# zerchen/AlignSDF

Measured on AMD Instinct MI355X. Metric: meshes_per_sec_hand_plus_obj_N256, higher is better.
Workload: dtype f32-class: 2 x f16 planes per operand (22 bit), 3 f16 MFMAs per product sum, f32 accumulate, every voxel <= 1e-5

## Files before the change

### alignsdf_amd/csrc/decoder.hip

```cpp
#include <hip/hip_runtime.h>

#include <cstdlib>
#include <cstring>
#include <new>
#include <vector>

#include "../../include/alignsdf_hip.h"
#include "common.h"
#include "pack.h"
#include "k1_launch.h"
#include "fold_kernels.h"
#include "sweep_kernels.h"

namespace asdf {
thread_local int g_last_hip_error = 0;
}

using namespace asdf;

struct asdf_decoder {
  asdf_decoder_spec_t spec;
  int device;
  int num_cus;
  float* stream;
  float* wlat;
  float* wpt;
  float* bias02;
  float* cst;
  int kp;
  float* embed;
  float* latent_stage;
  float* cls;
  int num_class;
  float* stream16;
  float* stream16_hi;
  float* cst16;
  float* a16;
  float* cst16p1;
  float* cst16p1_host;
  uint16_t* hi_host;
  uint16_t* hi_scaled;
  size_t hi_count;
  float s0p[ASDF_MAX_HEADS], s2p[ASDF_MAX_HEADS];
  int p1_usable;
  float s2[ASDF_MAX_HEADS];
  int math;
  bool sample_bound;
  int* status;
  float sw[ASDF_MAX_HEADS][3];
  float sx[ASDF_MAX_HEADS][3];
  float* cst_host;
  float* cst16_host;
  void* ev_start;
  void* ev_stop;
  float refine_tau;
  int* near_idx;
  int* near_count;
  unsigned char* band_mark;
  size_t band_mark_bytes;
  int* box_aux;
  int* band_idx;
  int* band_count;
  hipStream_t side;
  hipEvent_t ev_fork, ev_join;
  int audit_n;
  unsigned long long audit_seed;
  int* audit_rec;
  int* audit_idx;
  int* audit_count;
  int short_max;
  ShortParams shortp;
  hipStream_t audit_side;
  hipEvent_t ev_audit_fork, ev_audit_join;
  bool pixel_bound;
  PixelParams pixel;
  float* pa_proj;
  size_t pa_proj_floats;
  float* pa_cstb;
  float* pa_ws;
  float* pa_lat;
};
static constexpr int kShortClusters = kClusterCap / kWavePts * kHeads;
static constexpr int kNearCap = ASDF_NEAR_CAP;
static constexpr int kCandCap = ASDF_CAND_CAP;
static constexpr int kAuditCap = 1 << 18;
static constexpr int kCandDirect = 1 << 15;
static constexpr int kBandCap = ASDF_BAND_CAP;

static hipError_t rebuild_one_plane(asdf_decoder* d) {
  if (!d->stream16_hi || !d->hi_host) return hipSuccess;
  const CstOffsets co = cst_offsets(d->kp);
  const size_t n = (size_t)kHeads * co.floats;
  std::memcpy(d->cst16p1_host, d->cst_host, n * sizeof(float));
  d->p1_usable = 1;
  std::memcpy(d->hi_scaled, d->hi_host, d->hi_count * sizeof(uint16_t));
  for (int h = 0; h < d->spec.num_heads; ++h) {
    const float sx0 = d->sx[h][0], sx1 = d->sx[h][1], sx2 = d->sx[h][2];
    const float sw1p = 0.5f * sx1 / sx0, sw2p = 0.5f * sx2 / sx1, sw3 = d->sw[h][2];
    const float* c = d->cst_host + (size_t)h * co.floats;
    float* o = d->cst16p1_host + (size_t)h * co.floats;
    for (int i = 0; i < kTilesL1 * 32; ++i) o[co.b1 + i] = c[co.b1 + i] * (sw1p * sx0);
    const float s3 = sw3 * sx2;
    for (int i = 0; i < kHidden; ++i) { o[co.b3 + i] = c[co.b3 + i] * s3; o[co.w4 + i] = 0.5f * c[co.w4 + i] / s3; o[co.w4b + i] = 0.5f * c[co.w4b + i] / s3; }
    o[co.b4] = c[co.b4]; o[co.b4 + 1] = c[co.b4 + 1];
    o[co.b4 + 2] = o[co.b4 + 3] = o[co.b4 + 4] = 1.0f;
    d->s0p[h] = 0.5f * sx0;
    d->s2p[h] = sw2p * sx1;
    if (d->spec.feature_mode == ASDF_FEATURES_NERF) {
      for (int i = 0; i < kTilesHidden * d->kp * 64; ++i) { o[co.a0 + i] = c[co.a0 + i] * d->s0p[h]; o[co.a2 + i] = c[co.a2 + i] * d->s2p[h]; }
    }
    const float f[2] = {sw1p / d->sw[h][0], sw2p / d->sw[h][1]};
    for (int l = 0; l < 2; ++l) {
      uint16_t* rec = d->hi_scaled + ((size_t)h * 1024 + (size_t)l * 256) * 512;
      float top = 0.0f;
      for (size_t i = 0; i < (size_t)256 * 512; ++i) {
        _Float16 v;
        std::memcpy(&v, rec + i, 2);
        const float w = (float)v * f[l];
        top = std::fmax(top, std::fabs(w));
        v = (_Float16)w;
        std::memcpy(rec + i, &v, 2);
// ... 94 lines not shown

static int launch_decode(asdf_decoder_t* d, DecodeParams& p, hipStream_t st) {
  if (!d->sample_bound) return ASDF_EINVAL;
  p.stream = d->stream;
  p.cst = d->cst;
  p.status = d->status;
  p.first_mlp = 0;
  p.num_mlps = d->spec.num_heads;
  const bool two_out = d->spec.num_heads == 1;
  if (p.bbox) {
    hipLaunchKernelGGL(bbox_init_kernel, dim3(1), dim3(64), 0, st, p.bbox);
    ASDF_HIP(hipGetLastError());
  }
  const bool want_cls = p.logits || p.labels;
  if (d->pixel_bound && (want_cls || d->math != ASDF_MATH_F32 || p.mode == kGridSubset || two_out)) return ASDF_EINVAL;
  if (!two_out) {
    if (!p.sdf0 && !p.sdf1 && !want_cls) return ASDF_OK;
    if (!p.sdf1) p.num_mlps = 1;
    else if (!p.sdf0) { p.first_mlp = 1; p.num_mlps = 1; }
  }
  const long long ntiles = (p.P + kWgPts - 1) / kWgPts;
  if (ntiles == 0) return ASDF_OK;
  const int grid = (int)(ntiles < d->num_cus ? ntiles : d->num_cus);
  p.pf = d->spec.point_feats[0];
  if (p.logits || p.labels) {
    if (!d->cls) return ASDF_EINVAL;
    p.cls = d->cls;
    p.num_class = d->num_class;
    if (!two_out && p.first_mlp != 0) { p.first_mlp = 0; p.num_mlps = 2; }
    k1_cls_launch(d->kp, two_out, p, grid, st);
    ASDF_HIP(hipGetLastError());
    return ASDF_OK;
  }
  if (d->math == ASDF_MATH_F16X3 && d->stream16 && p.mode != kPointList) {
    p.stream = d->stream16;
    p.cst = d->cst16;
    ASDF_TRY(timed_launch(d, st, [&] { k1h_launch(d->kp, two_out, p, grid, st); }));
    if (d->refine_tau > 0.0f && p.P <= 0x7fffffffLL) {
      ASDF_HIP(hipMemsetAsync(d->near_count, 0, sizeof(int), st));
      ASDF_HIP(hipMemsetAsync(d->status + ASDF_STATUS_LIST_OVERFLOW, 0, 2 * sizeof(int), st));
      const long long n4 = (p.P + 3) / 4;
      const int cgrid = (int)((n4 + 255) / 256 < 2048 ? (n4 + 255) / 256 : 2048);
      hipLaunchKernelGGL(collect_near_level_kernel, dim3(cgrid), dim3(256), 0, st, p.sdf0, p.sdf1, p.P, d->refine_tau, d->near_idx,
                         d->near_count, kNearCap, d->status);
      int rgrid;
      DecodeParams q = list_params(d, p, d->stream, d->cst, d->near_idx, d->near_count, kNearCap, &rgrid);
      q.fixup_flag = p.bbox ? d->status + ASDF_STATUS_FIXUP : nullptr;
      ASDF_TRY(launch_subset(d, q, two_out, rgrid, st));
      if (p.bbox) {
        const int* flag = d->status + ASDF_STATUS_FIXUP;
        hipLaunchKernelGGL(bbox_reinit_keep_flags_kernel, dim3(1), dim3(64), 0, st, p.bbox, flag);
        const long long rows = (long long)p.N * p.N;
        const int bgrid = (int)((rows + 3) / 4 < 1024 ? (rows + 3) / 4 : 1024);
        if (p.sdf0) hipLaunchKernelGGL(neg_bbox_kernel, dim3(bgrid), dim3(256), 0, st, p.sdf0, p.N, p.N, p.N, p.bbox, flag);
        if (p.sdf1) hipLaunchKernelGGL(neg_bbox_kernel, dim3(bgrid), dim3(256), 0, st, p.sdf1, p.N, p.N, p.N, p.bbox + ASDF_BOX_STRIDE, flag);
        hipLaunchKernelGGL(near_overflow_to_bbox_kernel, dim3(1), dim3(64), 0, st, d->status, p.bbox);
      }
    }
  } else {
    ASDF_TRY(timed_launch(d, st, [&] {
      if (d->pixel_bound) k1pa_launch(p, d->pixel, grid, st);
      else k1_launch(d->kp, two_out, p, grid, st);
    }));
  }
  ASDF_HIP(hipGetLastError());
  return ASDF_OK;
}

// ... 76 lines not shown
  ASDF_TRY(one_plane_params(d, N, origin, voxel_size, lattice_dev, grid_mode, tau, sdf_hand_dev, sdf_obj_dev, rec_dev, p));
  const bool two_out = d->spec.num_heads == 1;
  hipStream_t st = (hipStream_t)stream;
  const long long P = p.P;
  if (!d->band_idx) {
    ASDF_HIP(hipMalloc((void**)&d->band_idx, 2 * (size_t)kBandCap * sizeof(int)));
    ASDF_HIP(hipMalloc((void**)&d->band_count, 2 * sizeof(int)));
  }
  if (d->band_mark_bytes < (size_t)P + 16) {
    if (d->band_mark) ASDF_HIP(hipFree(d->band_mark));
    d->band_mark = nullptr; d->band_mark_bytes = 0;
    ASDF_HIP(hipMalloc((void**)&d->band_mark, (size_t)P + 16));
    d->band_mark_bytes = (size_t)P + 16;
  }
  ASDF_TRY(one_plane_sweep(d, p, ClearRange{d->band_count, 2}, ClearRange{d->near_count, 1}, st));
  float* vols[2] = {sdf_hand_dev, sdf_obj_dev};
  for (int h = 0; h < (two_out ? 1 : 2); ++h) {
    if (!vols[h]) continue;
    ASDF_HIP(hipMemsetAsync(d->band_mark, 0, (size_t)P, st));
    const int per_slab = (((N - 1) + 3) >> 2) * (N - 1);
    const dim3 mgrid((per_slab + 255) / 256, N - 1 < 1024 ? N - 1 : 1024);
    hipLaunchKernelGGL(band_mark_kernel, mgrid, dim3(256), 0, st, vols[h], N, tau, d->band_mark);
    if (two_out) hipLaunchKernelGGL(band_mark_kernel, mgrid, dim3(256), 0, st, vols[1], N, tau, d->band_mark);
    const long long items = (P + 15) / 16;
    const int cgrid = (int)((items + 255) / 256 < 4096 ? (items + 255) / 256 : 4096);
    int* list = d->band_idx + (size_t)h * kBandCap;
    const bool publish = cgrid <= 256;
    int* audit_from = d->audit_rec + kAuditFrom + h;
    hipLaunchKernelGGL(band_compact_kernel, dim3(cgrid), dim3(256), 0, st, d->band_mark, P, list, d->band_count + h, kBandCap,
                       publish ? d->audit_rec + kAuditCompactDone + h : nullptr, audit_from);
    if (!publish) ASDF_HIP(hipMemcpyAsync(audit_from, d->band_count + h, sizeof(int), hipMemcpyDeviceToDevice, st));
    ASDF_TRY(enqueue_audit_picks(d, vols[h], two_out ? vols[1] : nullptr, d->band_mark, P, tau, list, d->band_count + h, kBandCap, h, st));
    int rgrid;
    DecodeParams q = list_params(d, p, d->stream16, d->cst16, list, d->band_count + h, kBandCap, &rgrid);
    q.bbox = nullptr; q.neg_thr = 0.0f;
    if (!two_out) { q.sdf0 = h == 0 ? vols[0] : nullptr; q.sdf1 = h == 1 ? vols[1] : nullptr; }
    q.first_mlp = two_out ? 0 : h; q.num_mlps = 1;
    q.audit = d->audit_n > 0 ? d->audit_rec : nullptr; q.audit_from = audit_from;
    k1h_subset_launch(d->kp, two_out, q, rgrid, st);
  }
  if (d->refine_tau > 0.0f) {
    for (int h = 0; h < 2; ++h)
      if (vols[h]) {
        const int l = two_out ? 0 : h;
        hipLaunchKernelGGL(collect_near_level_list_kernel, dim3(256), dim3(256), 0, st, vols[h], d->band_idx + (size_t)l * kBandCap,
                           d->band_count + l, kBandCap, d->refine_tau, d->near_idx, d->near_count, kNearCap, d->status);
      }
    int ngrid;
    DecodeParams q = list_params(d, p, d->stream, d->cst, d->near_idx, d->near_count, kNearCap, &ngrid);
    q.bbox = nullptr; q.neg_thr = 0.0f; q.status = nullptr;
    ASDF_TRY(launch_subset(d, q, two_out, ngrid, st));
  }
  hipLaunchKernelGGL(sweep_record_kernel, dim3(1), dim3(64), 0, st, rec_dev, d->status, d->near_count, d->audit_rec);
  ASDF_HIP(hipGetLastError());
  return ASDF_OK;
}

extern "C" {

int asdf_version(void) { return 130; }

int asdf_set_mfma_shape(int shape) {
  if (shape != 0 && shape != 16 && shape != 32) return ASDF_EINVAL;
  return k1h_set_shape(shape);
}
int asdf_get_mfma_shape(void) { return k1h_shape(); }

const char* asdf_strerror(int code) {
  switch (code) {
    case ASDF_OK: return "ok";
    case ASDF_EINVAL: return "invalid argument or unsupported decoder shape";
    case ASDF_ENOMEM: return "out of memory";
    case ASDF_EHIP: return "HIP runtime error";
    case ASDF_ENODEV: return "no gfx950 device";
    case ASDF_ENOSPC: return "buffer or workspace too small";
    case ASDF_ERANGE: return "Surface level must be within volume data range.";
    case ASDF_ENOSURF: return "No surface found at the given iso value.";
    default: return "unknown error";
  }
}

int asdf_last_hip_error(void) { return g_last_hip_error; }

int asdf_device_count(void) {
  int n = 0;
  if (hipGetDeviceCount(&n) != hipSuccess) return 0;
  int good = 0;
  for (int d = 0; d < n; ++d) {
    hipDeviceProp_t prop;
    if (hipGetDeviceProperties(&prop, d) == hipSuccess && std::strncmp(prop.gcnArchName, "gfx950", 6) == 0) ++good;
  }
  return good;
}

void asdf_decoder_destroy(asdf_decoder_t* d) {
  if (!d) return;
  for (hipStream_t side : {d->side, d->audit_side})
    if (side) { (void)hipStreamSynchronize(side); (void)hipStreamDestroy(side); }
  for (hipEvent_t ev : {d->ev_audit_fork, d->ev_audit_join, d->ev_fork, d->ev_join})
    if (ev) (void)hipEventDestroy(ev);
  void* bufs[] = {d->stream, d->wlat, d->wpt, d->bias02, d->cst, d->embed, d->cls, d->stream16, d->cst16, d->stream16_hi, d->a16, d->cst16p1,
                  d->pa_proj, d->pa_cstb, d->pa_ws, d->pa_lat, d->shortp.xchg, d->shortp.arrivals, d->band_mark, d->box_aux, d->band_idx,
                  d->band_count, d->status, d->latent_stage, d->near_idx, d->near_count, d->audit_rec, d->audit_idx, d->audit_count};
  for (void* b : bufs) (void)hipFree(b);
  std::free(d->cst_host);
  std::free(d->cst16_host);
  std::free(d->cst16p1_host);
  std::free(d->hi_host);
  std::free(d->hi_scaled);
  delete d;
}

int asdf_decoder_create(const asdf_decoder_spec_t* spec, const asdf_head_params_t* heads, asdf_decoder_t** out) {
  if (!spec || !heads || !out) return ASDF_EINVAL;
  *out = nullptr;
  if (!spec_supported(spec)) return ASDF_EINVAL;
  for (int h = 0; h < spec->num_heads; ++h) {
    if (spec->point_feats[h] < 1 || spec->point_feats[h] > ASDF_MAX_POINT_FEATS) return ASDF_EINVAL;
    if (kHidden - kLatent - spec->point_feats[h] < 1) return ASDF_EINVAL;
    for (int l = 0; l < 5; ++l)
      if (!heads[h].w[l] || !heads[h].b[l]) return ASDF_EINVAL;
  }
  int dev = 0;
  ASDF_HIP(hipGetDevice(&dev));
  hipDeviceProp_t prop;
  ASDF_HIP(hipGetDeviceProperties(&prop, dev));
  if (std::strncmp(prop.gcnArchName, "gfx950", 6) != 0) return ASDF_ENODEV;

  asdf_decoder* d = new (std::nothrow) asdf_decoder();
  if (!d) return ASDF_ENOMEM;
  std::memset(d, 0, sizeof(*d));
  d->spec = *spec;
  d->device = dev;
  d->num_cus = prop.multiProcessorCount;

  HostPack hp;
  if (!pack_decoder(*spec, heads, hp)) { delete d; return ASDF_ENOMEM; }
  d->kp = hp.kp;
  std::vector<float>&stream = hp.stream, &wlat = hp.wlat, &wpt = hp.wpt, &b02 = hp.b02, &cst = hp.cst, &emb = hp.emb;

  hipError_t e = hipSuccess;
  auto up = [&](float** dst, const std::vector<float>& src) {
    if (e != hipSuccess) return;
    e = hipMalloc((void**)dst, src.size() * sizeof(float));
    if (e == hipSuccess) e = hipMemcpy(*dst, src.data(), src.size() * sizeof(float), hipMemcpyHostToDevice);
  };
  up(&d->stream, stream); up(&d->wlat, wlat); up(&d->wpt, wpt); up(&d->bias02, b02); up(&d->cst, cst); up(&d->embed, emb);
  d->math = ASDF_MATH_F32;
  if (e == hipSuccess) {
    if (!pack_decoder_f16(*spec, heads, hp)) { asdf_decoder_destroy(d); return ASDF_ENOMEM; }
    up(&d->cst16, hp.cst16);
    if (e == hipSuccess) e = hipMalloc((void**)&d->stream16, (hp.stream16.size() + hp.stream16w.size()) * sizeof(uint16_t));
    if (e == hipSuccess) e = hipMemcpy(d->stream16, hp.stream16.data(), hp.stream16.size() * sizeof(uint16_t), hipMemcpyHostToDevice);
    if (e == hipSuccess) e = hipMemcpy(reinterpret_cast<uint16_t*>(d->stream16) + hp.stream16.size(), hp.stream16w.data(),
                                       hp.stream16w.size() * sizeof(uint16_t), hipMemcpyHostToDevice);
    if (e == hipSuccess) {
      const size_t nrec = hp.stream16.size() / 1024;
      std::vector<uint16_t> hi(nrec * 512);
      for (size_t r = 0; r < nrec; ++r) std::memcpy(&hi[r * 512], &hp.stream16[r * 1024], 512 * sizeof(uint16_t));
      e = hipMalloc((void**)&d->stream16_hi, hi.size() * sizeof(uint16_t));
      if (e == hipSuccess) e = hipMemcpy(d->stream16_hi, hi.data(), hi.size() * sizeof(uint16_t), hipMemcpyHostToDevice);
      d->hi_count = hi.size();
      d->hi_host = (uint16_t*)std::malloc(hi.size() * sizeof(uint16_t));
      d->hi_scaled = (uint16_t*)std::malloc(hi.size() * sizeof(uint16_t));
      d->cst16p1_host = (float*)std::malloc(hp.cst.size() * sizeof(float));
      if (!d->hi_host || !d->hi_scaled || !d->cst16p1_host) { asdf_decoder_destroy(d); return ASDF_ENOMEM; }
      std::memcpy(d->hi_host, hi.data(), hi.size() * sizeof(uint16_t));
      if (e == hipSuccess) e = hipMalloc((void**)&d->cst16p1, hp.cst.size() * sizeof(float));
      if (e == hipSuccess && d->kp == 2) {
        e = hipMalloc((void**)&d->a16, (size_t)kHeads * kA16Floats * sizeof(float));
        if (e == hipSuccess) e = hipMemset(d->a16, 0, (size_t)kHeads * kA16Floats * sizeof(float));
      }
    }
    for (int h = 0; h < kHeads; ++h) {
      d->s2[h] = h < spec->num_heads ? hp.s2[h] : 1.0f;
      for (int l = 0; l < 3; ++l) { d->sw[h][l] = h < spec->num_heads ? hp.sw[h][l] : 1.0f; d->sx[h][l] = kActScale; }
    }
    d->cst_host = (float*)std::malloc(hp.cst.size() * sizeof(float));
    d->cst16_host = (float*)std::malloc(hp.cst.size() * sizeof(float));
    if (!d->cst_host || !d->cst16_host) { asdf_decoder_destroy(d); return ASDF_ENOMEM; }
    std::memcpy(d->cst_host, hp.cst.data(), hp.cst.size() * sizeof(float));
    if (e == hipSuccess) e = rebuild_one_plane(d);
    if (e == hipSuccess) e = k1h_prepare();
    if (e == hipSuccess) e = k1s_nerf_prepare();
  }
  if (e == hipSuccess) e = k1_prepare();
  if (e == hipSuccess) e = k1_cls_prepare();
  if (e == hipSuccess) e = k1pa_prepare();
// ... 152 lines not shown

int asdf_decode_grid_dev(asdf_decoder_t* d, int32_t N, const float* lattice_dev, int32_t grid_mode,
                         float* sdf_hand_dev, float* sdf_obj_dev, int32_t* bbox_dev, void* stream) {
  if (!lattice_dev) return ASDF_EINVAL;
  return decode_grid_impl(d, N, nullptr, 0.0f, lattice_dev, grid_mode, sdf_hand_dev, sdf_obj_dev, bbox_dev, stream);
}

int asdf_zoom_cube(const int32_t* bbox_dev, int32_t N, float voxel_size, int32_t hand_branch, int32_t obj_branch, float* lattice_dev,
                   void* stream) {
  if (!bbox_dev || !lattice_dev || N < 2 || (!hand_branch && !obj_branch)) return ASDF_EINVAL;
  hipLaunchKernelGGL(zoom_cube_kernel, dim3(1), dim3(64), 0, (hipStream_t)stream, bbox_dev, N, voxel_size, hand_branch, obj_branch, lattice_dev);
  ASDF_HIP(hipGetLastError());
  return ASDF_OK;
}

int asdf_decode_grid_box(asdf_decoder_t* d, int32_t N, const float origin[3], float voxel_size, int32_t grid_mode, float tau,
                         float* scratch_hand_dev, float* scratch_obj_dev, int32_t* bbox_dev, void* stream) {
  if (!origin) return ASDF_EINVAL;
  DecodeParams p;
  ASDF_TRY(one_plane_params(d, N, origin, voxel_size, nullptr, grid_mode, tau, scratch_hand_dev, scratch_obj_dev, bbox_dev, p));
  const bool two_out = d->spec.num_heads == 1;
  hipStream_t st = (hipStream_t)stream;
  p.neg_thr = -tau;
  ASDF_TRY(one_plane_sweep(d, p, ClearRange{d->near_count, 1}, ClearRange{d->audit_count, 1}, st));
  bool audit_forked = false;
  struct AuditJoin {
    asdf_decoder* d; hipStream_t st; const bool* forked; bool done = false;
    void join() { if (*forked && !done) { done = true; (void)hipStreamWaitEvent(st, d->ev_audit_join, 0); } }
    ~AuditJoin() { join(); }
  } audit_join{d, st, &audit_forked};
  if (d->audit_n > 0) {
    ASDF_TRY(enqueue_audit_picks(d, p.sdf0, p.sdf1, nullptr, p.P, tau, d->audit_idx, d->audit_count, kAuditCap, 0, st));
    int agrid;
    DecodeParams a = list_params(d, p, d->stream16, d->cst16, d->audit_idx, d->audit_count, kAuditCap, &agrid);
    a.bbox = nullptr; a.neg_thr = 0.0f;
    a.audit = d->audit_rec; a.audit_from = nullptr;
    hipStream_t as = st;
    if (d->audit_side && !std::getenv("ASDF_AUDIT_INLINE")) {
      ASDF_HIP(hipEventRecord(d->ev_audit_fork, st));
      ASDF_HIP(hipStreamWaitEvent(d->audit_side, d->ev_audit_fork, 0));
      as = d->audit_side;
      audit_forked = true;
    }
    k1h_subset_launch(d->kp, two_out, a, agrid, as);
    if (audit_forked && hipEventRecord(d->ev_audit_join, d->audit_side) != hipSuccess) {
      (void)hipStreamSynchronize(d->audit_side);
      audit_forked = false;
      return ASDF_EHIP;
    }
  }
  const long long items = (N & 3) == 0 ? p.P / 4 : p.P;
  const int cgrid = (int)((items + 255) / 256 < 2048 ? (items + 255) / 256 : 2048);
  const bool direct_only = p.P <= 8LL * kCandDirect;
  const int cand_cap = direct_only ? kCandDirect : kCandCap;
  hipLaunchKernelGGL(collect_box_candidates_kernel, dim3(cgrid), dim3(256), 0, st, p.sdf0, p.sdf1, N, tau, p.bbox, d->near_idx,
                     d->near_count, cand_cap, d->status);
  if (!d->box_aux) ASDF_HIP(hipMalloc((void**)&d->box_aux, (4 + (size_t)kNearCap) * sizeof(int)));
  int* direct_count = d->box_aux, *twostep_count = d->box_aux + 1, *twostep_near = d->box_aux + 2, *twostep_idx = d->box_aux + 4;
  hipLaunchKernelGGL(split_candidate_count_kernel, dim3(1), dim3(64), 0, st, d->near_count, cand_cap, kCandDirect, d->box_aux);
  int rgrid;
  {
    DecodeParams q = list_params(d, p, d->stream, d->cst, d->near_idx, direct_count, kCandCap, &rgrid);
    q.fixup_flag = d->status + ASDF_STATUS_FIXUP;
    ASDF_TRY(launch_subset(d, q, two_out, rgrid, st));
  }
  if (!direct_only) {
    DecodeParams e = list_params(d, p, d->stream16, d->cst16, d->near_idx, twostep_count, kCandCap, &rgrid);
    e.bbox = nullptr; e.neg_thr = 0.0f;
    k1h_subset_launch(d->kp, two_out, e, rgrid, st);
    if (d->refine_tau > 0.0f) {
      const float* vols[2] = {p.sdf0, p.sdf1};
      for (int h = 0; h < 2; ++h)
        if (vols[h])
          hipLaunchKernelGGL(collect_near_level_list_kernel, dim3(256), dim3(256), 0, st, vols[h], d->near_idx, twostep_count, kCandCap,
                             d->refine_tau, twostep_idx, twostep_near, kNearCap, d->status);
      int ngrid;
      DecodeParams f = list_params(d, p, d->stream, d->cst, twostep_idx, twostep_near, kNearCap, &ngrid);
      f.bbox = nullptr; f.neg_thr = 0.0f; f.status = nullptr;
      ASDF_TRY(launch_subset(d, f, two_out, ngrid, st));
    }
    hipLaunchKernelGGL(extend_box_from_list_kernel, dim3(256), dim3(256), 0, st, p.sdf0, p.sdf1, d->near_idx, twostep_count, N, p.bbox);
  }
  audit_join.join();
  hipLaunchKernelGGL(sweep_record_kernel, dim3(1), dim3(64), 0, st, bbox_dev, d->status, d->near_count, d->audit_rec);
  ASDF_HIP(hipGetLastError());
  return ASDF_OK;
}

int asdf_decode_grid_band(asdf_decoder_t* d, int32_t N, const float origin[3], float voxel_size, int32_t grid_mode, float tau,
                          float* sdf_hand_dev, float* sdf_obj_dev, int32_t* rec_dev, void* stream) {
  if (!origin) return ASDF_EINVAL;
  return decode_grid_band_impl(d, N, origin, voxel_size, nullptr, grid_mode, tau, sdf_hand_dev, sdf_obj_dev, rec_dev, stream);
}

int asdf_decode_grid_band_dev(asdf_decoder_t* d, int32_t N, const float* lattice_dev, int32_t grid_mode, float tau,
                              float* sdf_hand_dev, float* sdf_obj_dev, int32_t* rec_dev, void* stream) {
  if (!lattice_dev) return ASDF_EINVAL;
  return decode_grid_band_impl(d, N, nullptr, 0.0f, lattice_dev, grid_mode, tau, sdf_hand_dev, sdf_obj_dev, rec_dev, stream);
}

// ... 6 lines not shown
}

int asdf_decoder_set_cluster_list(asdf_decoder_t* d, int32_t max_points) {
  if (!d || max_points < 0 || max_points > kClusterCap) return ASDF_EINVAL;
  d->shortp.cluster_max = max_points;
  if (max_points > 0 && d->shortp.fault) { ASDF_HIP(hipDeviceSynchronize()); ASDF_HIP(hipMemset(d->shortp.fault, 0, sizeof(int))); }
  return ASDF_OK;
}

int asdf_decoder_set_cluster_timeout(asdf_decoder_t* d, uint64_t ticks) {
  if (!d) return ASDF_EINVAL;
  d->shortp.timeout_ticks = ticks ? ticks : kClusterTimeoutTicks;
  return ASDF_OK;
}

int asdf_decoder_set_audit(asdf_decoder_t* d, int32_t voxels, uint64_t seed) {
  if (!d || voxels < 0 || voxels > kAuditCap) return ASDF_EINVAL;
  d->audit_n = voxels;
  d->audit_seed = seed;
  return ASDF_OK;
}

int asdf_decode_points(asdf_decoder_t* d, const float* xyz_dev, int64_t M, float* sdf_hand_dev, float* sdf_obj_dev,
                       void* stream) {
  if (!d || M < 0 || (M > 0 && !xyz_dev)) return ASDF_EINVAL;
  DecodeParams p;
  std::memset(&p, 0, sizeof(p));
  p.sdf0 = sdf_hand_dev; p.sdf1 = sdf_obj_dev; p.xyz = xyz_dev; p.P = M; p.N = 1; p.mode = kPointList;
  return launch_decode(d, p, (hipStream_t)stream);
}

int asdf_decoder_set_math(asdf_decoder_t* d, int32_t math) {
  if (!d || (math != ASDF_MATH_F32 && math != ASDF_MATH_F16X3)) return ASDF_EINVAL;
  if (math == ASDF_MATH_F16X3 && (!d->stream16 || d->pixel_bound)) return ASDF_EINVAL;
  d->math = math;
  return ASDF_OK;
}

int asdf_decoder_get_math(const asdf_decoder_t* d) { return d ? d->math : ASDF_EINVAL; }

int asdf_decoder_time_next_sweep(asdf_decoder_t* d, void* event_start, void* event_stop) {
  if (!d || (!event_start) != (!event_stop)) return ASDF_EINVAL;
  d->ev_start = event_start;
  d->ev_stop = event_stop;
  return ASDF_OK;
}

int asdf_decoder_set_refine(asdf_decoder_t* d, float tau) {
  if (!d || !(tau >= 0.0f) || tau > 1.0f) return ASDF_EINVAL;
  d->refine_tau = tau;
  return ASDF_OK;
}

int asdf_decoder_status(asdf_decoder_t* d, int32_t out_host[16], int32_t clear, void* stream) {
  if (!d || !out_host) return ASDF_EINVAL;
  hipStream_t st = (hipStream_t)stream;
  ASDF_HIP(hipMemcpyAsync(out_host, d->status, ASDF_STATUS_WORDS * sizeof(int), hipMemcpyDeviceToHost, st));
  if (clear) {
    ASDF_HIP(hipMemsetAsync(d->status, 0, ASDF_STATUS_CLUSTER_FAULT * sizeof(int), st));
    ASDF_HIP(hipMemsetAsync(d->status + ASDF_STATUS_CLUSTER_FAULT + 1, 0, (ASDF_STATUS_WORDS - ASDF_STATUS_CLUSTER_FAULT - 1) * sizeof(int), st));
  }
  ASDF_HIP(hipStreamSynchronize(st));
  return ASDF_OK;
}

int asdf_decoder_get_act_scales(const asdf_decoder_t* d, float sx_out[ASDF_MAX_HEADS][3]) {
  if (!d || !sx_out) return ASDF_EINVAL;
// ... 64 lines not shown
```

### alignsdf_amd/csrc/sdf_mlp_f16w_kernel.h

```cpp
#pragma once
#include "sdf_mlp_f16_kernel.h"

namespace asdf {

static_assert(ASDF16_STAGE_KB == 16 && ASDF16_MIX_SPLIT && ASDF16_EPI_STEPS && ASDF16_DMA_PER_KB && ASDF16_PRELOAD && ASDF16_LOADS_FIRST &&
                  ASDF16_PIN_ACC,
              "the W form is written for the shipped schedule of the split-half kernel");

#define ASDF_MFMA16W(a, b, c) __builtin_amdgcn_mfma_f32_16x16x32_f16((a), (b), (c), 0, 0, 0)
#define ASDF_MFMA4W(a, b, c) __builtin_amdgcn_mfma_f32_16x16x4f32((a), (b), (c), 0, 0, 0)

__device__ __forceinline__ f32x4 acc_get4(const f32x16& a, int o) {
  f32x4 v;
  v[0] = a[o]; v[1] = a[o + 1]; v[2] = a[o + 2]; v[3] = a[o + 3];
  return v;
}
__device__ __forceinline__ void acc_set4(f32x16& a, int o, const f32x4& v) { a[o] = v[0]; a[o + 1] = v[1]; a[o + 2] = v[2]; a[o + 3] = v[3]; }

__device__ __forceinline__ f32x16 load_bias16w(const float* tile_words, int lane) {
  const int q = lane >> 4;
  const float* w0 = tile_words + (q & 1) * 16 + 4 * (q >> 1);
  int dup = 0;
  asm volatile("" : "+v"(dup));
  const float* w1 = w0 + dup;
  f32x16 r;
  acc_set4(r, 0, *reinterpret_cast<const f32x4*>(w0)); acc_set4(r, 4, *reinterpret_cast<const f32x4*>(w0 + 8));
  acc_set4(r, 8, *reinterpret_cast<const f32x4*>(w1)); acc_set4(r, 12, *reinterpret_cast<const f32x4*>(w1 + 8));
  return r;
}

__device__ __forceinline__ void pin_acc_w(f32x16& acc) {
#pragma unroll
  for (int o = 0; o < 16; o += 4) {
    f32x4 q;
    q[0] = acc[o]; q[1] = acc[o + 1]; q[2] = acc[o + 2]; q[3] = acc[o + 3];
    asm volatile("" : "+a"(q));
    acc[o] = q[0]; acc[o + 1] = q[1]; acc[o + 2] = q[2]; acc[o + 3] = q[3];
  }
}

#ifndef ASDF16_W_M0_CLOBBER
#define ASDF16_W_M0_CLOBBER 1
#endif
template <int P>
__device__ __forceinline__ void dma_piece_w(const float* src, unsigned dst) {
#if ASDF16_W_M0_CLOBBER
  asm volatile(
      "s_mov_b32 m0, %1\n\t"
      "s_nop 0\n\t"
      "global_load_lds_dwordx4 %0, off offset:%c2"
      :
      : "v"(src + (P >> 2) * 1024), "s"(dst + (P >> 2) * 4096), "i"((P & 3) * 1024)
      : "memory", "m0");
#else
  dma_piece<P>(src, dst);
#endif
}

template <int KB, int Q, int SLOT, int ABL, class Pre, class Epi>
__device__ __forceinline__ void stage16w(f32x16& acc, const h8 (&xh)[KB], const h8 (&xl)[KB], const float* ring, const float* next_src,
                                         unsigned lds_ring_base, int lane, int wave, h8 (&ah)[S16<2>::kPrefetch], h8 (&al)[S16<2>::kPrefetch],
                                         Pre&& pre, Epi&& epi) {
  using SG = S16<2>;
  constexpr int PF = SG::kPrefetch;
  constexpr int BKB = ASDF16_BARRIER_KB;
  constexpr int nslot = (SLOT + kRing - 1) % kRing;
  static_assert(KB == 32 || KB == 16, "records per tile");
  static_assert(kS16Kb - BKB >= SG::kPieces, "one LDS-DMA piece per record behind the barrier");
  const float* src = next_src + wave * SG::kWaveFloats + lane * 4;
  const unsigned dst = lds_ring_base + (nslot * SG::kFloats + wave * SG::kWaveFloats) * 4;
  const h8* cur = reinterpret_cast<const h8*>(ring + SLOT * SG::kFloats) + lane;
  const h8* nxt = reinterpret_cast<const h8*>(ring + ((SLOT + 1) % kRing) * SG::kFloats) + lane;
  h8 bufh[kS16Kb + PF], bufl[kS16Kb + PF];
#pragma unroll
  for (int i = 0; i < PF; ++i) { bufh[i] = ah[i]; bufl[i] = al[i]; }
#pragma unroll
  for (int kb = 0; kb < kS16Kb; ++kb) {
    if (kb == BKB && !(ABL & 1)) {
      asm volatile("s_waitcnt vmcnt(8)" ::: "memory");
      if (!(ABL & 16)) __builtin_amdgcn_s_barrier();
    }
    bufh[kb + PF] = kb + PF < kS16Kb ? cur[((kb + PF) * 2 + 0) * 64] : nxt[((kb + PF - kS16Kb) * 2 + 0) * 64];
    bufl[kb + PF] = kb + PF < kS16Kb ? cur[((kb + PF) * 2 + 1) * 64] : nxt[((kb + PF - kS16Kb) * 2 + 1) * 64];
    pre(kb);
    __builtin_amdgcn_sched_barrier(0);
    const int ri = Q * kS16Kb + kb;
    const int xb = KB == 32 ? 2 * (ri % 16) : (ri & ~1), o = (KB == 32 ? ri / 16 : (ri & 1)) * 4;
    const bool snake = ri & 1;
    const int xa = xb + (snake ? 1 : 0), xc = xb + (snake ? 0 : 1);
#pragma unroll
    for (int j = 0; j < 3; ++j) {
      f32x4 s0 = acc_get4(acc, o), s1 = acc_get4(acc, 8 + o);
      f32x4& sa = snake ? s1 : s0;
      f32x4& sb = snake ? s0 : s1;
      if (j == 0) { sa = ASDF_MFMA16W(bufh[kb], xl[xa], sa); sa = ASDF_MFMA16W(bufl[kb], xh[xa], sa); }
      if (j == 1) { sa = ASDF_MFMA16W(bufh[kb], xh[xa], sa); sb = ASDF_MFMA16W(bufh[kb], xl[xc], sb); }
      if (j == 2) { sb = ASDF_MFMA16W(bufl[kb], xh[xc], sb); sb = ASDF_MFMA16W(bufh[kb], xh[xc], sb); }
      acc_set4(acc, o, s0); acc_set4(acc, 8 + o, s1);
      const int m = j == 2 ? kb - BKB : -1;
      if (!(ABL & 1) && !(ABL & 32) && m >= 0 && m < SG::kPieces) {
        if (m == 0) dma_piece_w<0>(src, dst);
        else if (m == 1) dma_piece_w<1>(src, dst);
        else if (m == 2) dma_piece_w<2>(src, dst);
        else if (m == 3) dma_piece_w<3>(src, dst);
        else if (m == 4) dma_piece_w<4>(src, dst);
        else if (m == 5) dma_piece_w<5>(src, dst);
        else if (m == 6) dma_piece_w<6>(src, dst);
        else dma_piece_w<7>(src, dst);
        __builtin_amdgcn_sched_barrier(0);
      }
      epi(kb, j);
      __builtin_amdgcn_sched_barrier(0);
    }
    __builtin_amdgcn_sched_barrier(0);
  }
#pragma unroll
  for (int i = 0; i < PF; ++i) { ah[i] = bufh[kS16Kb + i]; al[i] = bufl[kS16Kb + i]; }
}

template <int ABL = 0, bool SUB = false>
__device__ __forceinline__ void sdf_mlp_f16w_body(const DecodeParams& p) {
  using CL = CstLayout<2>;
  using SG = S16<2>;
  static_assert(lds_bytes_f16(2, 2) <= 160 * 1024, "LDS budget");
  extern __shared__ __attribute__((aligned(16))) float smem[];
  float* ring = smem;
  float* cst = smem + SG::kRingFloats;

  const int tid = threadIdx.x;
  const int lane = tid & 63;
  const int wave = __builtin_amdgcn_readfirstlane(tid >> 6);
  const int half = lane >> 5;

  float lat_vs = p.vs, lat_o0 = p.o0, lat_o1 = p.o1, lat_o2 = p.o2;
  if (p.lattice) { lat_o0 = p.lattice[0]; lat_o1 = p.lattice[1]; lat_o2 = p.lattice[2]; lat_vs = p.lattice[3]; }
  long long npts = p.P;
  if (SUB) { const long long c = *p.count_dev; npts = c < npts ? c : npts; }
  const long long ntiles = (npts + kWgPts - 1) / kWgPts;
  if ((long long)blockIdx.x >= ntiles) return;

  const unsigned lds_ring_base = (unsigned)(size_t)(__attribute__((address_space(3))) float*)ring;
  if (!SUB && p.status && p.mode != kPointList && blockIdx.x == 0 && tid == 0) reinterpret_cast<long long*>(p.status + ASDF_STATUS_CLOCK)[0] = clock64();

#pragma unroll 1
  for (int slot = 0; slot < p.num_mlps; ++slot) {
    const int head = p.first_mlp + slot;
    const float* hc = cst;
    int* wrec = reinterpret_cast<int*>(cst + CL::kFloats) + wave * kWrecInts;
    if (lane < kWrecInts) wrec[lane] = lane >= 16 ? 0 : ((lane & 7) < 3 ? 0x7fffffff : ((lane & 7) < 6 ? -1 : 0));
    asm volatile("s_waitcnt vmcnt(0)" ::: "memory");
    __syncthreads();
    {
      const f32x4* src4 = reinterpret_cast<const f32x4*>(p.cst + (size_t)head * CL::kFloats);
      for (int i = tid; i < CL::kFloats / 4; i += 256) reinterpret_cast<f32x4*>(cst)[i] = src4[i];
    }
    const float* sbase0 = p.stream + (size_t)kStagesAll * kStageFloats + (size_t)head * kS16Head * SG::kFloats;
#pragma unroll
    for (int s = 0; s < ((ABL & 33) ? kRing : kRing - 1); ++s) {
      const float* src = sbase0 + (size_t)s * SG::kFloats + wave * SG::kWaveFloats + lane * 4;
      const unsigned dst = lds_ring_base + (s * SG::kFloats + wave * SG::kWaveFloats) * 4;
#pragma unroll
      for (int c = 0; c < SG::kPieces; ++c) lds_dma16(src + c * 256, dst + c * 1024);
    }
    if (ABL & 33) asm volatile("s_waitcnt vmcnt(0)" ::: "memory");
    asm volatile("s_waitcnt vmcnt(16)" ::: "memory");
    __syncthreads();
    h8 ah[SG::kPrefetch], al[SG::kPrefetch];
#pragma unroll
    for (int i = 0; i < SG::kPrefetch; ++i) {
      ah[i] = (reinterpret_cast<const h8*>(ring) + lane)[(i * 2 + 0) * 64];
      al[i] = (reinterpret_cast<const h8*>(ring) + lane)[(i * 2 + 1) * 64];
    }
    const float mul1 = hc[CL::kB4 + 2], mul2 = hc[CL::kB4 + 3], mul0 = hc[CL::kB4 + 4];
    int audit_from = 0x7fffffff;
    if (SUB && p.audit) audit_from = p.audit_from ? *p.audit_from : 0;
    auto bias_at = [&](int off, int t) -> f32x16 { return load_bias16w(hc + off + t * 32, lane); };
    auto pt_word = [&](int off, int t, int fh) -> float {
      return hc[off + (t * 2 + (lane >> 5)) * 64 + ((lane >> 4) & 1) * 32 + 16 * fh + (lane & 15)];
    };

#pragma unroll 1
    for (long long tile = blockIdx.x; tile < ntiles; tile += gridDim.x) {
      const long long pi = tile * kWgPts + wave * kWavePts + (lane & 31);
      const bool valid = pi < npts;
      const long long po = SUB ? (valid ? (long long)p.idx[pi] : 0) : pi;
      float x0 = 0.f, x1 = 0.f, x2 = 0.f;
      if (SUB) {
        grid_point(po, p.N, p.grid_mode, lat_vs, lat_o0, lat_o1, lat_o2, x0, x1, x2);
      } else if (p.mode == kPointList) {
        if (valid) { x0 = p.xyz[pi * 3 + 0]; x1 = p.xyz[pi * 3 + 1]; x2 = p.xyz[pi * 3 + 2]; }
      } else {
        grid_point(valid ? pi : 0, p.N, p.mode, lat_vs, lat_o0, lat_o1, lat_o2, x0, x1, x2);
      }
      float amax = 0.0f, amax1 = 0.0f, amax2 = 0.0f;
      float bq[2];
// ... 22 lines not shown
      float pf2[2];
      float w4c[2], w4n[2];
      constexpr int kPreKb = ASDF16_PRE_KB;
      static_assert(kPreKb >= kEpiShift + kEpiChunks, "preload K-block inside the epilogue slots");
      auto load_pf2 = [&](int t) { pf2[0] = pt_word(CL::kA2, t, 0); pf2[1] = pt_word(CL::kA2, t, 1); };
      auto load_w4 = [&](int t, int c) {
        const int wq = lane >> 4;
        const float* w4 = hc + CL::kW4 + (t * 2 + (wq & 1)) * 16 + 4 * (2 * ((c >> 1) & 1) + (wq >> 1)) + 2 * (c & 1);
        w4n[0] = w4[0]; w4n[1] = w4[1];
      };
      auto next_w4 = [&]() { w4c[0] = w4n[0]; w4c[1] = w4n[1]; };

      h8 h0h[2 * kTilesHidden], h0l[2 * kTilesHidden];
      f32x16 acc0[2];
      float pf0[2][2];
      auto l0_load = [&](int t) {
        acc0[t & 1] = bias_at(CL::kC0, t);
        pf0[t & 1][0] = pt_word(CL::kA0, t, 0); pf0[t & 1][1] = pt_word(CL::kA0, t, 1);
      };
      constexpr int kL0Front = kS16Kb / 2;
      l0_load(0);
      acc1[0] = bias_at(CL::kB1, 0);
#pragma unroll
      for (int t = 0; t < kL0Front; ++t) {
        l0_load(t + 1);
        __builtin_amdgcn_sched_barrier(0);
        f32x16 acc = acc0[t & 1];
        pt_mfma(acc, pf0[t & 1]);
        split_tile<2, 1, true>(acc, acc, mul0, h0h[2 * t], h0l[2 * t], h0h[2 * t + 1], h0l[2 * t + 1], amax);
        __builtin_amdgcn_sched_barrier(0);
      }

#define ASDF_STAGE16W(KB, Q, SLOT, ACC, XH, XL, SIDX, PRE, EPI) \
  stage16w<KB, Q, SLOT, ABL>(ACC, XH, XL, ring, src_of((SIDX) + 3), lds_ring_base, lane, wave, ah, al, PRE, EPI)

      float er[2] = {0.0f, 0.0f};
      h8 h1h[2 * kTilesL1], h1l[2 * kTilesL1];
      if (ABL & 4) for (int t = 0; t < 2 * kTilesL1; ++t) { h1h[t] = h0h[t]; h1l[t] = h0l[t]; }
#pragma unroll
      for (int t = 0; t < kTilesL1; ++t) {
        f32x16& acc = acc1[t & 1];
        auto pre = [&](int kb) {
          const int c = kb - kEpiShift;
          if (t == 0 && c >= 0 && c + 1 < kEpiChunks) l0_load(kL0Front + c + 1);
        };
        auto epi = [&](int kb, int g) {
          const int c = kb - kEpiShift;
          if (c < 0 || c >= kEpiChunks) return;
          if (t == 0) {
            const int T = kL0Front + c;
            if (g == 0) pt_mfma(acc0[T & 1], pf0[T & 1]);
#pragma unroll
            for (int e = 0; e < 8; ++e)
              if (e / 3 == g) split_part<2, 1, true>(acc0[T & 1], acc0[T & 1], mul0, h0h[2 * T], h0l[2 * T], h0h[2 * T + 1], h0l[2 * T + 1], amax, e);
            return;
          }
          if (ABL & 4) { asm volatile("" :: "v"(acc1[(t - 1) & 1])); return; }
          if (g == 0) pin_acc_w(acc1[(t - 1) & 1]);
          split_part<2, 1, true>(acc1[(t - 1) & 1], acc1[(t - 1) & 1], mul1, h1h[2 * (t - 1)], h1l[2 * (t - 1)], h1h[2 * (t - 1) + 1],
                                 h1l[2 * (t - 1) + 1], amax1, c, -1, g, er);
        };
        auto pre_last = [&](int c) {
          if (c != kPreKb) return;
          if (t + 1 < kTilesL1) acc1[(t + 1) & 1] = bias_at(CL::kB1, t + 1);
          else { acc2[0] = bias_at(CL::kC2, 0); load_pf2(0); }
        };
        if (t & 1) {
// ... 193 lines not shown
```

Before: 13.67.

## Use SGPR-base addressing for LDS-DMA weight loads and upload only needed half stream

The wide f16 kernel's LDS-DMA weight loads now use a scalar base address plus one per-lane VGPR offset computed once, instead of a full 64-bit per-lane address for each piece. This frees vector registers and removes per-piece address arithmetic. The host now uploads only the stream image the chosen kernel shape needs and defers the other to a lazy upload on first use. The wide image is now indexed from its own base instead of at an offset inside a combined buffer. The risk is a blocking host copy if the other form is ever requested, and reliance on the m0 save/restore inline assembly being correct.

```diff
diff --git a/alignsdf_amd/csrc/decoder.hip b/alignsdf_amd/csrc/decoder.hip
--- a/alignsdf_amd/csrc/decoder.hip
+++ b/alignsdf_amd/csrc/decoder.hip
@@ -33,6 +33,9 @@
   float* cls;
   int num_class;
   float* stream16;
+  float* stream16w;
+  uint16_t* stream16_pending;
+  size_t stream16_halves;
   float* stream16_hi;
   float* cst16;
   float* a16;
@@ -87,6 +90,21 @@
 static constexpr int kCandDirect = 1 << 15;
 static constexpr int kBandCap = ASDF_BAND_CAP;
 
+static bool has_split_half(const asdf_decoder* d) { return d->stream16 || d->stream16w; }
+static int split_half_stream(asdf_decoder* d, bool two_out, const float** out) {
+  const bool wide = d->kp == 2 && !two_out && k1h_shape() == 16;
+  float** img = wide ? &d->stream16w : &d->stream16;
+  if (!*img) {
+    if (!d->stream16_pending) return ASDF_EINVAL;
+    ASDF_HIP(hipMalloc((void**)img, d->stream16_halves * sizeof(uint16_t)));
+    ASDF_HIP(hipMemcpy(*img, d->stream16_pending, d->stream16_halves * sizeof(uint16_t), hipMemcpyHostToDevice));
+    std::free(d->stream16_pending);
+    d->stream16_pending = nullptr;
+  }
+  *out = *img;
+  return ASDF_OK;
+}
+
 static hipError_t rebuild_one_plane(asdf_decoder* d) {
   if (!d->stream16_hi || !d->hi_host) return hipSuccess;
   const CstOffsets co = cst_offsets(d->kp);
@@ -247,8 +265,8 @@
     ASDF_HIP(hipGetLastError());
     return ASDF_OK;
   }
-  if (d->math == ASDF_MATH_F16X3 && d->stream16 && p.mode != kPointList) {
-    p.stream = d->stream16;
+  if (d->math == ASDF_MATH_F16X3 && has_split_half(d) && p.mode != kPointList) {
+    ASDF_TRY(split_half_stream(d, two_out, &p.stream));
     p.cst = d->cst16;
     ASDF_TRY(timed_launch(d, st, [&] { k1h_launch(d->kp, two_out, p, grid, st); }));
     if (d->refine_tau > 0.0f && p.P <= 0x7fffffffLL) {
@@ -391,7 +409,9 @@
     if (!publish) ASDF_HIP(hipMemcpyAsync(audit_from, d->band_count + h, sizeof(int), hipMemcpyDeviceToDevice, st));
     ASDF_TRY(enqueue_audit_picks(d, vols[h], two_out ? vols[1] : nullptr, d->band_mark, P, tau, list, d->band_count + h, kBandCap, h, st));
     int rgrid;
-    DecodeParams q = list_params(d, p, d->stream16, d->cst16, list, d->band_count + h, kBandCap, &rgrid);
+    const float* s16;
+    ASDF_TRY(split_half_stream(d, two_out, &s16));
+    DecodeParams q = list_params(d, p, s16, d->cst16, list, d->band_count + h, kBandCap, &rgrid);
     q.bbox = nullptr; q.neg_thr = 0.0f;
     if (!two_out) { q.sdf0 = h == 0 ? vols[0] : nullptr; q.sdf1 = h == 1 ? vols[1] : nullptr; }
     q.first_mlp = two_out ? 0 : h; q.num_mlps = 1;
@@ -458,7 +478,7 @@
     if (side) { (void)hipStreamSynchronize(side); (void)hipStreamDestroy(side); }
   for (hipEvent_t ev : {d->ev_audit_fork, d->ev_audit_join, d->ev_fork, d->ev_join})
     if (ev) (void)hipEventDestroy(ev);
-  void* bufs[] = {d->stream, d->wlat, d->wpt, d->bias02, d->cst, d->embed, d->cls, d->stream16, d->cst16, d->stream16_hi, d->a16, d->cst16p1,
+  void* bufs[] = {d->stream, d->wlat, d->wpt, d->bias02, d->cst, d->embed, d->cls, d->stream16, d->stream16w, d->cst16, d->stream16_hi, d->a16, d->cst16p1,
                   d->pa_proj, d->pa_cstb, d->pa_ws, d->pa_lat, d->shortp.xchg, d->shortp.arrivals, d->band_mark, d->box_aux, d->band_idx,
                   d->band_count, d->status, d->latent_stage, d->near_idx, d->near_count, d->audit_rec, d->audit_idx, d->audit_count};
   for (void* b : bufs) (void)hipFree(b);
@@ -467,6 +487,7 @@
   std::free(d->cst16p1_host);
   std::free(d->hi_host);
   std::free(d->hi_scaled);
+  std::free(d->stream16_pending);
   delete d;
 }
 
@@ -509,10 +530,21 @@
   if (e == hipSuccess) {
     if (!pack_decoder_f16(*spec, heads, hp)) { asdf_decoder_destroy(d); return ASDF_ENOMEM; }
     up(&d->cst16, hp.cst16);
-    if (e == hipSuccess) e = hipMalloc((void**)&d->stream16, (hp.stream16.size() + hp.stream16w.size()) * sizeof(uint16_t));
-    if (e == hipSuccess) e = hipMemcpy(d->stream16, hp.stream16.data(), hp.stream16.size() * sizeof(uint16_t), hipMemcpyHostToDevice);
-    if (e == hipSuccess) e = hipMemcpy(reinterpret_cast<uint16_t*>(d->stream16) + hp.stream16.size(), hp.stream16w.data(),
-                                       hp.stream16w.size() * sizeof(uint16_t), hipMemcpyHostToDevice);
+    {
+      const bool w_form = d->kp == 2 && spec->num_heads != 1;
+      const bool wide = w_form && k1h_shape() == 16;
+      const std::vector<uint16_t>& now = wide ? hp.stream16w : hp.stream16;
+      const std::vector<uint16_t>& later = wide ? hp.stream16 : hp.stream16w;
+      float** img = wide ? &d->stream16w : &d->stream16;
+      d->stream16_halves = now.size();
+      if (e == hipSuccess) e = hipMalloc((void**)img, now.size() * sizeof(uint16_t));
+      if (e == hipSuccess) e = hipMemcpy(*img, now.data(), now.size() * sizeof(uint16_t), hipMemcpyHostToDevice);
+      if (w_form) {
+        d->stream16_pending = (uint16_t*)std::malloc(later.size() * sizeof(uint16_t));
+        if (!d->stream16_pending) { asdf_decoder_destroy(d); return ASDF_ENOMEM; }
+        std::memcpy(d->stream16_pending, later.data(), later.size() * sizeof(uint16_t));
+      }
+    }
     if (e == hipSuccess) {
       const size_t nrec = hp.stream16.size() / 1024;
       std::vector<uint16_t> hi(nrec * 512);
@@ -731,7 +763,9 @@
   if (d->audit_n > 0) {
     ASDF_TRY(enqueue_audit_picks(d, p.sdf0, p.sdf1, nullptr, p.P, tau, d->audit_idx, d->audit_count, kAuditCap, 0, st));
     int agrid;
-    DecodeParams a = list_params(d, p, d->stream16, d->cst16, d->audit_idx, d->audit_count, kAuditCap, &agrid);
+    const float* s16;
+    ASDF_TRY(split_half_stream(d, two_out, &s16));
+    DecodeParams a = list_params(d, p, s16, d->cst16, d->audit_idx, d->audit_count, kAuditCap, &agrid);
     a.bbox = nullptr; a.neg_thr = 0.0f;
     a.audit = d->audit_rec; a.audit_from = nullptr;
     hipStream_t as = st;
@@ -764,7 +798,9 @@
     ASDF_TRY(launch_subset(d, q, two_out, rgrid, st));
   }
   if (!direct_only) {
-    DecodeParams e = list_params(d, p, d->stream16, d->cst16, d->near_idx, twostep_count, kCandCap, &rgrid);
+    const float* s16;
+    ASDF_TRY(split_half_stream(d, two_out, &s16));
+    DecodeParams e = list_params(d, p, s16, d->cst16, d->near_idx, twostep_count, kCandCap, &rgrid);
     e.bbox = nullptr; e.neg_thr = 0.0f;
     k1h_subset_launch(d->kp, two_out, e, rgrid, st);
     if (d->refine_tau > 0.0f) {
@@ -837,7 +873,7 @@
 
 int asdf_decoder_set_math(asdf_decoder_t* d, int32_t math) {
   if (!d || (math != ASDF_MATH_F32 && math != ASDF_MATH_F16X3)) return ASDF_EINVAL;
-  if (math == ASDF_MATH_F16X3 && (!d->stream16 || d->pixel_bound)) return ASDF_EINVAL;
+  if (math == ASDF_MATH_F16X3 && (!has_split_half(d) || d->pixel_bound)) return ASDF_EINVAL;
   d->math = math;
   return ASDF_OK;
 }
diff --git a/alignsdf_amd/csrc/sdf_mlp_f16w_kernel.h b/alignsdf_amd/csrc/sdf_mlp_f16w_kernel.h
--- a/alignsdf_amd/csrc/sdf_mlp_f16w_kernel.h
+++ b/alignsdf_amd/csrc/sdf_mlp_f16w_kernel.h
@@ -42,32 +42,59 @@
 #ifndef ASDF16_W_M0_CLOBBER
 #define ASDF16_W_M0_CLOBBER 1
 #endif
+#ifndef ASDF16_W_SADDR
+#define ASDF16_W_SADDR 1
+#endif
 template <int P>
-__device__ __forceinline__ void dma_piece_w(const float* src, unsigned dst) {
-#if ASDF16_W_M0_CLOBBER
+__device__ __forceinline__ void dma_piece_w(const float* base, unsigned voff, unsigned dst) {
+#if ASDF16_W_M0_CLOBBER && ASDF16_W_SADDR
+  asm volatile(
+      "s_mov_b32 m0, %1\n\t"
+      "s_nop 0\n\t"
+      "global_load_lds_dwordx4 %0, %2 offset:%c3"
+      :
+      : "v"(voff), "s"(dst + (P >> 2) * 4096), "s"(base + (P >> 2) * 1024), "i"((P & 3) * 1024)
+      : "memory", "m0");
+#elif ASDF16_W_M0_CLOBBER
   asm volatile(
       "s_mov_b32 m0, %1\n\t"
       "s_nop 0\n\t"
       "global_load_lds_dwordx4 %0, off offset:%c2"
       :
-      : "v"(src + (P >> 2) * 1024), "s"(dst + (P >> 2) * 4096), "i"((P & 3) * 1024)
+      : "v"(base + (voff >> 2) + (P >> 2) * 1024), "s"(dst + (P >> 2) * 4096), "i"((P & 3) * 1024)
       : "memory", "m0");
 #else
-  dma_piece<P>(src, dst);
+  dma_piece<P>(base + (voff >> 2), dst);
+#endif
+}
+template <int P>
+__device__ __forceinline__ void dma_piece_w_keep(const float* base, unsigned voff, unsigned dst) {
+#if ASDF16_W_SADDR
+  unsigned keep;
+  asm volatile(
+      "s_mov_b32 %0, m0\n\t"
+      "s_mov_b32 m0, %2\n\t"
+      "s_nop 0\n\t"
+      "global_load_lds_dwordx4 %1, %3 offset:%c4\n\t"
+      "s_mov_b32 m0, %0"
+      : "=&s"(keep)
+      : "v"(voff), "s"(dst + (P >> 2) * 4096), "s"(base + (P >> 2) * 1024), "i"((P & 3) * 1024)
+      : "memory");
+#else
+  lds_dma16(base + (voff >> 2) + P * 256, dst + P * 1024);
 #endif
 }
 
 template <int KB, int Q, int SLOT, int ABL, class Pre, class Epi>
 __device__ __forceinline__ void stage16w(f32x16& acc, const h8 (&xh)[KB], const h8 (&xl)[KB], const float* ring, const float* next_src,
-                                         unsigned lds_ring_base, int lane, int wave, h8 (&ah)[S16<2>::kPrefetch], h8 (&al)[S16<2>::kPrefetch],
-                                         Pre&& pre, Epi&& epi) {
+                                         unsigned voff, unsigned lds_ring_base, int lane, int wave, h8 (&ah)[S16<2>::kPrefetch],
+                                         h8 (&al)[S16<2>::kPrefetch], Pre&& pre, Epi&& epi) {
   using SG = S16<2>;
   constexpr int PF = SG::kPrefetch;
   constexpr int BKB = ASDF16_BARRIER_KB;
   constexpr int nslot = (SLOT + kRing - 1) % kRing;
   static_assert(KB == 32 || KB == 16, "records per tile");
   static_assert(kS16Kb - BKB >= SG::kPieces, "one LDS-DMA piece per record behind the barrier");
-  const float* src = next_src + wave * SG::kWaveFloats + lane * 4;
   const unsigned dst = lds_ring_base + (nslot * SG::kFloats + wave * SG::kWaveFloats) * 4;
   const h8* cur = reinterpret_cast<const h8*>(ring + SLOT * SG::kFloats) + lane;
   const h8* nxt = reinterpret_cast<const h8*>(ring + ((SLOT + 1) % kRing) * SG::kFloats) + lane;
@@ -99,14 +126,14 @@
       acc_set4(acc, o, s0); acc_set4(acc, 8 + o, s1);
       const int m = j == 2 ? kb - BKB : -1;
       if (!(ABL & 1) && !(ABL & 32) && m >= 0 && m < SG::kPieces) {
-        if (m == 0) dma_piece_w<0>(src, dst);
-        else if (m == 1) dma_piece_w<1>(src, dst);
-        else if (m == 2) dma_piece_w<2>(src, dst);
-        else if (m == 3) dma_piece_w<3>(src, dst);
-        else if (m == 4) dma_piece_w<4>(src, dst);
-        else if (m == 5) dma_piece_w<5>(src, dst);
-        else if (m == 6) dma_piece_w<6>(src, dst);
-        else dma_piece_w<7>(src, dst);
+        if (m == 0) dma_piece_w<0>(next_src, voff, dst);
+        else if (m == 1) dma_piece_w<1>(next_src, voff, dst);
+        else if (m == 2) dma_piece_w<2>(next_src, voff, dst);
+        else if (m == 3) dma_piece_w<3>(next_src, voff, dst);
+        else if (m == 4) dma_piece_w<4>(next_src, voff, dst);
+        else if (m == 5) dma_piece_w<5>(next_src, voff, dst);
+        else if (m == 6) dma_piece_w<6>(next_src, voff, dst);
+        else dma_piece_w<7>(next_src, voff, dst);
         __builtin_amdgcn_sched_barrier(0);
       }
       epi(kb, j);
@@ -140,6 +167,8 @@
   if ((long long)blockIdx.x >= ntiles) return;
 
   const unsigned lds_ring_base = (unsigned)(size_t)(__attribute__((address_space(3))) float*)ring;
+  unsigned voff = (wave * SG::kWaveFloats + lane * 4) * 4;
+  asm volatile("" : "+v"(voff));
   if (!SUB && p.status && p.mode != kPointList && blockIdx.x == 0 && tid == 0) reinterpret_cast<long long*>(p.status + ASDF_STATUS_CLOCK)[0] = clock64();
 
 #pragma unroll 1
@@ -152,15 +181,18 @@
     __syncthreads();
     {
       const f32x4* src4 = reinterpret_cast<const f32x4*>(p.cst + (size_t)head * CL::kFloats);
-      for (int i = tid; i < CL::kFloats / 4; i += 256) reinterpret_cast<f32x4*>(cst)[i] = src4[i];
-    }
-    const float* sbase0 = p.stream + (size_t)kStagesAll * kStageFloats + (size_t)head * kS16Head * SG::kFloats;
+      int i0 = tid;
+      asm volatile("" : "+v"(i0));
+      for (int i = i0; i < CL::kFloats / 4; i += 256) reinterpret_cast<f32x4*>(cst)[i] = src4[i];
+    }
+    const float* sbase0 = p.stream + (size_t)head * kS16Head * SG::kFloats;
 #pragma unroll
     for (int s = 0; s < ((ABL & 33) ? kRing : kRing - 1); ++s) {
-      const float* src = sbase0 + (size_t)s * SG::kFloats + wave * SG::kWaveFloats + lane * 4;
+      const float* src = sbase0 + (size_t)s * SG::kFloats;
       const unsigned dst = lds_ring_base + (s * SG::kFloats + wave * SG::kWaveFloats) * 4;
-#pragma unroll
-      for (int c = 0; c < SG::kPieces; ++c) lds_dma16(src + c * 256, dst + c * 1024);
+      static_assert(SG::kPieces == 8, "a wave's share of a stage");
+      dma_piece_w_keep<0>(src, voff, dst); dma_piece_w_keep<1>(src, voff, dst); dma_piece_w_keep<2>(src, voff, dst); dma_piece_w_keep<3>(src, voff, dst);
+      dma_piece_w_keep<4>(src, voff, dst); dma_piece_w_keep<5>(src, voff, dst); dma_piece_w_keep<6>(src, voff, dst); dma_piece_w_keep<7>(src, voff, dst);
     }
     if (ABL & 33) asm volatile("s_waitcnt vmcnt(0)" ::: "memory");
     asm volatile("s_waitcnt vmcnt(16)" ::: "memory");
@@ -249,7 +281,7 @@
       }
 
 #define ASDF_STAGE16W(KB, Q, SLOT, ACC, XH, XL, SIDX, PRE, EPI) \
-  stage16w<KB, Q, SLOT, ABL>(ACC, XH, XL, ring, src_of((SIDX) + 3), lds_ring_base, lane, wave, ah, al, PRE, EPI)
+  stage16w<KB, Q, SLOT, ABL>(ACC, XH, XL, ring, src_of((SIDX) + 3), voff, lds_ring_base, lane, wave, ah, al, PRE, EPI)
 
       float er[2] = {0.0f, 0.0f};
       h8 h1h[2 * kTilesL1], h1l[2 * kTilesL1];
```

Measured after the change: 13.67 (median of 2 runs). No clear change (-0.0%).
